# fpusan/moira

Measured on AMD Instinct MI355X. Metric: reads/sec filtered (300 bp synthetic), higher is better.
Workload: dtype f64; 1 GPU; BASELINE configs[1]: 10000000 synthetic single-end 300 bp reads, poisson_binomial filter, alpha 0.005, uncert 0.01, resident in HBM (uint8 10000000 x 320, seed 2); reads_per_gpu=10000000, read_length=300, row_stride=320, parallelism=host-side split, 1 rank(s), no data-path collective, world_size=1, mode=bit-exact (no FMA)

## Files before the change

### include/moira_pb.h

```cpp
#ifndef MOIRA_PB_H
#define MOIRA_PB_H

#include <stdint.h>

#ifdef __cplusplus
extern "C" {
#endif
#if defined(__GNUC__) || defined(__clang__)
#pragma GCC visibility push(default)
#endif

#define MPB_OK            0
#define MPB_E_INVALID    -1
#define MPB_E_NODEVICE   -2
#define MPB_E_HIP        -3
#define MPB_E_NOMEM      -4
#define MPB_E_RANGE      -5

#define MPB_AMBIG_TREAT_AS_ERRORS 0
#define MPB_AMBIG_IGNORE          1
#define MPB_AMBIG_DISALLOW        2

#define MPB_FLAG_ROUND      1u
#define MPB_FLAG_FAST_FMA   2u
#define MPB_FLAG_ODDS      128u
#define MPB_FLAG_DECISION_ONLY 8u
#define MPB_FLAG_TEST_UNDERPREDICT 4u
#define MPB_FLAG_COUNT_CELLS 32u
#define MPB_FLAG_BATCHED_ONLY 16u

#define MPB_FLAG_NO_NARROW 64u
#define MPB_FLAG_NARROW_ROWS(r) (((uint32_t)(r) & 15u) << 8)

#define MPB_FLAG_NARROW_SPLIT(c) (((uint32_t)(c) & 255u) << 12)

#define MPB_FLAG_ODDS_NARROW (1u << 20)

#define MPB_FLAG_POISSON_DEVICE_TAIL (1u << 21)

#define MPB_K_PREPASS   0
#define MPB_K_SCAN      1
#define MPB_K_SCATTER   2
#define MPB_K_DP        3
#define MPB_K_OVERFLOW  4
#define MPB_K_LAMBDA    5
#define MPB_K_WIDE      6
#define MPB_K_NARROW    7
#define MPB_K_FALLBACK  8
#define MPB_K_SAMPLE    9
#define MPB_K_POISSON_TAIL 10
#define MPB_K_PACK_TEXT 11
#define MPB_K_CONTIG    12
#define MPB_K_CONTIG_ROWS 13
#define MPB_K_BGZF_DEFLATE 14
#define MPB_K_BGZF_SCAN  15
#define MPB_K_BGZF_FRAME 16
#define MPB_K_BGZF_INFLATE 17
#define MPB_K_FQ_LINES  18
#define MPB_K_FQ_SCAN   19
#define MPB_K_FQ_STARTS 20
#define MPB_K_FQ_ROWS   21
#define MPB_K_COUNT     22

typedef struct mpb_ctx mpb_ctx;

typedef struct mpb_filter_params {
    double   alpha;
    double   uncert;
    double   maxerrors;
    int32_t  ambig_mode;
    uint32_t flags;
} mpb_filter_params;

typedef struct mpb_filter_counts {
    int64_t n_reads;
    int64_t n_pass;
    int64_t n_fail;
    int64_t n_overflow;
} mpb_filter_counts;

const char *mpb_version(void);
const char *mpb_last_error(void);
int mpb_device_count(void);

int mpb_create(int device_id, mpb_ctx **out);
int mpb_destroy(mpb_ctx *ctx);
int mpb_host_lut(double *a_out, double *b_out);
int mpb_device_lut(mpb_ctx *ctx, double *a_out, double *b_out);
int mpb_stream(mpb_ctx *ctx, void **stream_out);
int mpb_synchronize(mpb_ctx *ctx);

int mpb_malloc(mpb_ctx *ctx, int64_t bytes, void **dptr_out);
int mpb_free(mpb_ctx *ctx, void *dptr);
int mpb_memcpy_h2d(mpb_ctx *ctx, void *dst_dev, const void *src_host, int64_t bytes);
int mpb_memcpy_d2h(mpb_ctx *ctx, void *dst_host, const void *src_dev, int64_t bytes);
int mpb_memset(mpb_ctx *ctx, void *dst_dev, int value, int64_t bytes);
int mpb_host_alloc(mpb_ctx *ctx, int64_t bytes, void **hptr_out);
int mpb_host_free(mpb_ctx *ctx, void *hptr);

int mpb_pack_read(const char *seq, const int32_t *quals, int32_t len,
                  uint8_t *row_out, int32_t row_bytes);
int mpb_pack_read_ascii(const char *seq, const char *qual_ascii, int32_t len,
                        int32_t offset, uint8_t *row_out, int32_t row_bytes);

int mpb_pack_batch_ascii(const char *seq_cat, const char *qual_cat, const int64_t *off, int64_t n,
                         int32_t fastq_offset, int32_t max_len, int64_t row_stride,
                         uint8_t *out, int32_t *lens_out);

int mpb_decode_ascii_device(mpb_ctx *ctx, const uint8_t *d_seq, const uint8_t *d_qual_ascii, int64_t n,
                            int64_t row_stride, const int32_t *d_len, int32_t fixed_len,
                            int32_t fastq_offset, uint8_t *d_q_out, int32_t *d_err);

int mpb_encode_ascii_device(mpb_ctx *ctx, const uint8_t *d_q, int64_t n, int64_t row_stride, int32_t fastq_offset,
                            uint8_t *d_seq_out, uint8_t *d_qual_out);

#define MPB_IDX_SEQ_OFF  2
#define MPB_IDX_QUAL_OFF 4
#define MPB_IDX_QUAL_LEN 5
#define MPB_IDX_COLS     6

typedef struct mpb_text_row { int64_t seq_off, qual_off; int32_t len, pad; } mpb_text_row;
// ... 206 lines not shown
```

### moira_amd/_lib.py

```python
import ctypes as C
import os

_HERE = os.path.dirname(os.path.abspath(__file__))
LIB_PATH = os.path.join(_HERE, "libmoira_pb.so")

MAX_LEN = 65535
OK, E_INVALID, E_NODEVICE, E_HIP, E_NOMEM, E_RANGE = 0, -1, -2, -3, -4, -5
AMBIG = {"treat_as_errors": 0, "ignore": 1, "disallow": 2}
FLAG_ROUND, FLAG_FAST_FMA, FLAG_TEST_UNDERPREDICT, FLAG_DECISION_ONLY, FLAG_BATCHED_ONLY, FLAG_COUNT_CELLS = 1, 2, 4, 8, 16, 32
FLAG_NO_NARROW = 64
FLAG_ODDS = 128
FLAG_ODDS_NARROW = 1 << 20
FLAG_POISSON_DEVICE_TAIL = 1 << 21


def FLAG_NARROW_ROWS(r):
    return (int(r) & 15) << 8


K_PREPASS, K_SCAN, K_SCATTER, K_DP, K_OVERFLOW, K_LAMBDA, K_WIDE, K_NARROW, K_FALLBACK, K_SAMPLE = 0, 1, 2, 3, 4, 5, 6, 7, 8, 9
K_POISSON_TAIL = 10
K_PACK_TEXT = 11
KERNEL_NAMES = {K_PREPASS: "prepass", K_SCAN: "scan", K_SCATTER: "scatter", K_DP: "dp", K_OVERFLOW: "overflow", K_LAMBDA: "lambda",
                K_WIDE: "wide", K_NARROW: "narrow", K_FALLBACK: "fallback", K_SAMPLE: "sample", K_POISSON_TAIL: "poisson_tail",
                K_PACK_TEXT: "pack_text"}
K_CONTIG, K_CONTIG_ROWS = 12, 13
CONTIG_KERNEL_NAMES = {K_CONTIG: "contig", K_CONTIG_ROWS: "contig_rows"}
K_BGZF_DEFLATE, K_BGZF_SCAN, K_BGZF_FRAME = 14, 15, 16
BGZF_KERNEL_NAMES = {K_BGZF_DEFLATE: "bgzf_deflate", K_BGZF_SCAN: "bgzf_scan", K_BGZF_FRAME: "bgzf_frame"}
K_BGZF_INFLATE = 17
INFLATE_KERNEL_NAMES = {K_BGZF_INFLATE: "bgzf_inflate"}
K_FQ_LINES, K_FQ_SCAN, K_FQ_STARTS, K_FQ_ROWS = 18, 19, 20, 21
INDEX_KERNEL_NAMES = {K_FQ_LINES: "fq_lines", K_FQ_SCAN: "fq_scan", K_FQ_STARTS: "fq_starts", K_FQ_ROWS: "fq_rows"}
FQ_WHY = ("taken", "non-ASCII byte", "lone carriage return", "line table", "row check")
BGZF_WHY = ("ok", "header", "block type", "stored length", "code-length code", "repeat", "tree", "symbol", "distance", "overrun",
            "short", "truncated", "trailing bytes", "crc")
BGZF_DATA = 0xff00


class MoiraPBError(RuntimeError):
    pass


class NoDeviceError(MoiraPBError):
    pass


class FilterParams(C.Structure):
    _fields_ = [("alpha", C.c_double), ("uncert", C.c_double), ("maxerrors", C.c_double),
                ("ambig_mode", C.c_int32), ("flags", C.c_uint32)]


class PathInfo(C.Structure):
    _fields_ = [("narrow_rows", C.c_int32), ("sampled", C.c_int32), ("n_fallback", C.c_int64),
                ("sample_hist", C.c_int32 * 16), ("narrow_split", C.c_int32), ("narrow_waves", C.c_int32)]


class FilterCounts(C.Structure):
    _fields_ = [("n_reads", C.c_int64), ("n_pass", C.c_int64), ("n_fail", C.c_int64),
                ("n_overflow", C.c_int64)]


class TextRow(C.Structure):
    _fields_ = [("seq_off", C.c_int64), ("qual_off", C.c_int64), ("len", C.c_int32), ("pad", C.c_int32)]


class PairRow(C.Structure):
    _fields_ = [("fseq_off", C.c_int64), ("fqual_off", C.c_int64), ("fhdr_off", C.c_int64), ("rseq_off", C.c_int64),
                ("rqual_off", C.c_int64), ("l1", C.c_int32), ("l2", C.c_int32), ("hdr_len", C.c_int32), ("pad", C.c_int32)]


class ContigParams(C.Structure):
    _fields_ = [(k, C.c_int32) for k in ("match", "mismatch", "gap", "insert", "deltaq", "consensus", "qscore_cap", "trim_overlap")]


class BgzfStats(C.Structure):
    _fields_ = [(k, C.c_int64) for k in ("members", "dynamic", "fixed", "stored", "literals", "matches", "matched_bytes")]


class BgzfMemberRow(C.Structure):
    _fields_ = [("stream_off", C.c_int64), ("out_off", C.c_int64), ("stream_len", C.c_int32), ("out_len", C.c_int32)]


class BgzfInflateStats(C.Structure):
    _fields_ = [(k, C.c_int64) for k in ("members", "taken", "handed_back", "stored_blocks", "fixed_blocks", "dynamic_blocks",
                                         "literals", "matches", "matched_bytes", "longest_code")]


CONTIG_MAX_LEN = 384

_VP, _I32P, _U8P, _DP = C.c_void_p, C.POINTER(C.c_int32), C.POINTER(C.c_uint8), C.POINTER(C.c_double)
PROTOTYPES = {
    "mpb_version": (C.c_char_p, []),
    "mpb_last_error": (C.c_char_p, []),
    "mpb_device_count": (C.c_int, []),
    "mpb_create": (C.c_int, [C.c_int, C.POINTER(_VP)]),
# ... 136 lines not shown
```

### moira_amd/build.py

```python
import fcntl
import hashlib
import os
import subprocess
import sys

HERE = os.path.dirname(os.path.abspath(__file__))
ROOT = os.path.dirname(HERE)
CSRC = os.path.join(HERE, "csrc")
LIB = os.path.join(HERE, "libmoira_pb.so")
HOST_SOURCES = [os.path.join(CSRC, name) for name in ("mpb_hostonly.cpp", "mpb_context.cpp", "mpb_resident.cpp", "mpb_hostfed.cpp",
                                                      "mpb_perread.cpp", "mpb_poisson.cpp", "mpb_text.cpp", "mpb_contig.cpp",
                                                      "mpb_bgzf.cpp", "mpb_inflate.cpp", "mpb_index.cpp", "mpb_broker.cpp")]
CONTIG_KERNELS = os.path.join(CSRC, "mpb_contig_kernels.hip")
BGZF_KERNELS = os.path.join(CSRC, "mpb_bgzf_kernels.hip")
INFLATE_KERNELS = os.path.join(CSRC, "mpb_inflate_kernels.hip")
INDEX_KERNELS = os.path.join(CSRC, "mpb_index_kernels.hip")
SOURCES = [os.path.join(CSRC, "mpb_kernels.hip"), CONTIG_KERNELS, BGZF_KERNELS, INFLATE_KERNELS, INDEX_KERNELS] + HOST_SOURCES
DEPS = SOURCES + [os.path.join(CSRC, "mpb_internal.h"), os.path.join(CSRC, "mpb_host_internal.h"),
                  os.path.join(CSRC, "mpb_shared.h"), os.path.join(CSRC, "mpb_hostonly.h"), os.path.join(CSRC, "mpb_ctx.h"),
                  os.path.join(CSRC, "mpb_dp_tiles.inc"),
                  os.path.join(CSRC, "mpb_narrow_ring.inc"), os.path.join(CSRC, "mpb_narrow_rs.inc"),
                  os.path.join(CSRC, "mpb_narrow_rg.inc"),
                  os.path.join(CSRC, "mpb_contig_lane.inc"), os.path.join(CSRC, "mpb_contig_args.h"),
                  os.path.join(CSRC, "mpb_contig_rows.inc"),
                  os.path.join(CSRC, "mpb_bgzf_lane.inc"),
                  os.path.join(CSRC, "mpb_inflate_lane.inc"),
                  os.path.join(CSRC, "mpb_index_lane.inc"),
                  os.path.join(CSRC, "contig_posterior.h"),
                  os.path.join(CSRC, "libmoira_pb.map"),
                  os.path.join(ROOT, "include", "moira_pb.h"),
                  os.path.join(ROOT, "include", "mpb_synth.h")]
HIPCC = os.environ.get("HIPCC", "/opt/rocm/bin/hipcc")
FLAGS = ["-O3", "--offload-arch=gfx950", "-fPIC", "-shared", "-std=c++17",
         "-ffp-contract=off", "-fno-fast-math", "-pthread", "-Wall", "-Wno-unused-function",
         "-Werror=pass-failed",
         "-fvisibility=hidden",
         "-Wl,--version-script=" + os.path.join(CSRC, "libmoira_pb.map"),
         "-x", "hip"]


CONTIG_LIB = os.path.join(HERE, "libmoira_contig.so")
CONTIG_SRC = os.path.join(CSRC, "contig.cpp")
CXX = os.environ.get("CXX", "g++")


CONTIG_DEPS = [CONTIG_SRC, os.path.join(CSRC, "contig_posterior.h"), os.path.join(ROOT, "include", "moira_contig.h"),
               os.path.join(ROOT, "include", "moira_io.h")]


def _digest(paths, flags):
    h = hashlib.sha256(" ".join(flags).encode())
    for p in paths:
        with open(p, "rb") as f:
            h.update(f.read())
    return h.hexdigest()


def _is_stale(lib, deps, flags):
    stamp = lib + ".stamp"
    if not os.path.exists(lib) or not os.path.exists(stamp):
        return True
    try:
        return open(stamp).read().strip() != _digest(deps, flags)
    except OSError:
        return True


def _locked_build(lib, deps, flags, cmd, force, verbose):
    with open(lib + ".lock", "w") as lk:
        fcntl.flock(lk, fcntl.LOCK_EX)
        try:
            if force or _is_stale(lib, deps, flags):
                if verbose:
                    print(" ".join(cmd))
                tmp = lib + ".tmp.%d" % os.getpid()
                subprocess.check_call(cmd[:-1] + [tmp])
                os.replace(tmp, lib)
                with open(lib + ".stamp", "w") as f:
                    f.write(_digest(deps, flags))
                if verbose:
                    print("%s: COMPILED now (sources + flags digest %s)" % (os.path.basename(lib), _digest(deps, flags)[:16]))
            elif verbose:
                print("%s: up to date" % os.path.basename(lib))
        finally:
            fcntl.flock(lk, fcntl.LOCK_UN)
    return lib


def report(lib, deps, flags):
    state = "STALE" if _is_stale(lib, deps, flags) else "up to date: its stamp equals the digest of its sources + flags"
    print("%s: %s (digest %s, %d bytes)" % (os.path.basename(lib), state, _digest(deps, flags)[:16],
                                            os.path.getsize(lib) if os.path.exists(lib) else 0))


CONTIG_FLAGS = ["-O3", "-fPIC", "-shared", "-std=c++17", "-ffp-contract=off", "-pthread", "-Wall"]


def contig_stale():
    return _is_stale(CONTIG_LIB, CONTIG_DEPS, CONTIG_FLAGS)


def build_contig(force=False, verbose=False):
    if not force and not contig_stale():
        return CONTIG_LIB
    cmd = [CXX] + CONTIG_FLAGS + [CONTIG_SRC, "-o", CONTIG_LIB]
# ... 46 lines not shown
```

### moira_amd/csrc/mpb_kernels.hip

```cpp

#include "mpb_internal.h"
#include <cstdlib>
#include <cstdio>
#include "../../include/mpb_synth.h"

#pragma clang fp contract(off)

__shared__ double2 mpb_s_lut[256];
__shared__ unsigned long long mpb_s_cells;

namespace {

__constant__ MpbClass c_classes[MPB_NCLS] = MPB_CLASS_TABLE;

struct ClassOfRows {
    uint8_t t[MPB_TILE_MAX_ROWS + 1];
    constexpr ClassOfRows() : t{}
    {
        constexpr MpbClass cl[MPB_NCLS] = MPB_CLASS_TABLE;
        for (int rows = 0; rows < MPB_TILE_MAX_ROWS + 1; rows++) {
            int c = 0;
            for (int k = 0; k < MPB_NCLS - 1; k++) c += (rows > cl[k].cap) ? 1 : 0;
            t[rows] = (uint8_t)c;
        }
// ... 1656 lines not shown
        js = hit ? r : js;
        acc = na;
    }
    if (!(js >= 0 && p0 >= 0x1p-900)) return false;
    e = mpb_add_ns(prm, cross_ee_odds(true, js, prm.thr, p0, lo, hi), nsv);
    if (mode_unsure(prm, e, li)) return false;
    keep = mpb_round_and_keep(prm, e, nsv > 0, li);
    return true;
}

template <int AR = MPB_AR_EXACT, int R>
__device__ __forceinline__ NarRead nar_finish(double (&v)[R], uint32_t &nonzero, const MpbDevParams &prm, bool valid, bool good,
                                              int li, int64_t i, int32_t *my_seg, int &nlist, int lane)
{
    NarRead o;
    if constexpr (AR == MPB_AR_ODDS) {
        o.nsv = li - (int)nonzero;
        o.done = good && nar_odds_result(v, prm, o.nsv, li, o.e, o.keep);
    } else {
    double acc = 0.0, lo = 0.0, hi = 0.0;
    int js = -1;
#pragma unroll
    for (int r = 0; r < R; r++) {
        const double na = acc + v[r];
        const bool hit = (js < 0) && (na > prm.thr);
        lo = hit ? acc : lo;
        hi = hit ? na : hi;
        js = hit ? r : js;
        acc = na;
    }
    o.done = good && js >= 0;
    o.nsv = li - (int)nonzero;
    if (o.done) o.keep = read_result(prm, true, js, lo, hi, o.nsv, o.nsv > 0, li, o.e);
    }
    const unsigned long long todo = __ballot(valid && !o.done);
    if (todo) {
        if (valid && !o.done) my_seg[nlist + __popcll(todo & ((1ull << lane) - 1ull))] = (int32_t)i;
        nlist += __popcll(todo);
    }
#pragma unroll
    for (int r = 0; r < R; r++) v[r] = r == 0 ? 1.0 : 0.0;
    nonzero = 0;
    return o;
}

#define MPB_NRS_TILE 8192
__device__ __forceinline__ void nar_tile_lane(int lane, int &wr_even, int &wr_odd, int &x0)
{
    const int r8 = lane >> 3, c8 = lane & 7;
    wr_even = r8 * 128 + ((c8 ^ (r8 >> 1)) << 4);
    wr_odd = r8 * 128 + ((c8 ^ (4 + (r8 >> 1))) << 4);
    x0 = lane * 128 + (((lane >> 1) & 7) << 4);
}
__device__ __forceinline__ void nar_tile_write(uint8_t *tile, int wr_even, int wr_odd, const u32x4 (&pre)[8])
{
#pragma unroll
    for (int j = 0; j < 8; j++) *reinterpret_cast<u32x4 *>(tile + j * 1024 + ((j & 1) ? wr_odd : wr_even)) = pre[j];
}
__device__ __forceinline__ void nar_tile_fence()
{
    __builtin_amdgcn_fence(__ATOMIC_RELEASE, "wavefront");
    __builtin_amdgcn_wave_barrier();
    __builtin_amdgcn_fence(__ATOMIC_ACQUIRE, "wavefront");
}


#define MPB_NAR_AR MPB_AR_EXACT
#define MPB_NAR_RLO RLO

template <int R, int D>
__global__ __launch_bounds__(256) void k_narrow(const uint8_t *__restrict__ q, int64_t n, int64_t stride, int32_t li,
                                                MpbDevParams prm, const double2 *__restrict__ lut_g,
                                                double *__restrict__ ee, int32_t *__restrict__ ns, uint8_t *__restrict__ pass,
                                                int32_t *__restrict__ seg, int32_t *__restrict__ wave_count)
#include "mpb_narrow_ring.inc"

template <int R, bool ALIGNED>
__global__ __launch_bounds__(256) void k_narrow_rs(const uint8_t *__restrict__ q, int64_t n, int64_t stride, int32_t li, int32_t k,
                                                   MpbDevParams prm, const double2 *__restrict__ lut_g,
                                                   double *__restrict__ ee, int32_t *__restrict__ ns, uint8_t *__restrict__ pass,
                                                   int32_t *__restrict__ seg, int32_t *__restrict__ wave_count)
#include "mpb_narrow_rs.inc"

#define MPB_RG_WIN 4096
#define MPB_RG_BINS 64

__device__ __forceinline__ int rg_group_cost(int chunks) { return chunks + ((chunks + 7) >> 3) + 2; }

__device__ __forceinline__ uint32_t rg_block_excl_scan(uint32_t x, uint32_t *s_wave, int tid)
{
    const int lane = tid & 63, w = tid >> 6;
    uint32_t incl = x;
#pragma unroll
    for (int off = 1; off < 64; off <<= 1) {
        const uint32_t y = __shfl_up(incl, off);
        if (lane >= off) incl += y;
    }
    if (lane == 63) s_wave[w] = incl;
    __syncthreads();
    uint32_t base = 0;
#pragma unroll
    for (int k = 0; k < 3; k++) base += k < w ? s_wave[k] : 0;
    __syncthreads();
    return base + incl - x;
}

__global__ __launch_bounds__(256) void k_rag_sort(const int32_t *__restrict__ len, int64_t n, int32_t max_len, int key_shift,
                                                  int32_t split, int32_t low_pct,
                                                  int2 *__restrict__ ord, int32_t *__restrict__ gpre,
                                                  unsigned long long *__restrict__ wsum)
{
    __shared__ __attribute__((aligned(16))) uint16_t s_cnt[8 * 256];
    __shared__ __attribute__((aligned(16))) uint16_t s_idx[2][MPB_RG_WIN];
    __shared__ __attribute__((aligned(16))) uint16_t s_len[MPB_RG_WIN];
    __shared__ uint32_t s_wave[4];
    const int tid = threadIdx.x, lane = tid & 63, w = tid >> 6;
    const int64_t w0 = (int64_t)blockIdx.x * MPB_RG_WIN;
    const int m = (int)min((int64_t)MPB_RG_WIN, n - w0);
#pragma unroll
    for (int k = 0; k < 16; k++) {
        const int i = k * 256 + tid;
        const int l = i < m ? len[w0 + i] : 0;
        s_len[i] = (uint16_t)((l < 0 || l > max_len) ? 0xffff : l);
    }
    __syncthreads();
    auto key_of = [key_shift](uint32_t l) { return l == 0xffffu ? 0u : ((l + 15u) >> 4) >> key_shift; };
    uint32_t el[16];
    {
        const u32x4 a = *reinterpret_cast<const u32x4 *>(s_len + 16 * tid), b = *reinterpret_cast<const u32x4 *>(s_len + 16 * tid + 8);
        const uint32_t ww[8] = {a.x, a.y, a.z, a.w, b.x, b.y, b.z, b.w};
#pragma unroll
        for (int e = 0; e < 8; e++) { el[2 * e] = key_of(ww[e] & 0xffffu); el[2 * e + 1] = key_of(ww[e] >> 16); }
    }
    const int mine = min(16, max(0, m - 16 * tid));
#pragma unroll
    for (int pass = 0; pass < 2; pass++) {
        if (pass == 1) {
            __syncthreads();
            const u32x4 a = *reinterpret_cast<const u32x4 *>(s_idx[0] + 16 * tid), b = *reinterpret_cast<const u32x4 *>(s_idx[0] + 16 * tid + 8);
            const uint32_t ww[8] = {a.x, a.y, a.z, a.w, b.x, b.y, b.z, b.w};
#pragma unroll
            for (int e = 0; e < 8; e++) { el[2 * e] = ww[e] & 0xffffu; el[2 * e + 1] = ww[e] >> 16; }
        }
        unsigned long long c_lo = 0, c_hi = 0;
#pragma unroll
        for (int r = 0; r < 16; r++) {
            const int d = pass == 0 ? (int)(el[r] & 7u) : (int)(el[r] >> 12);
            const unsigned long long inc = r < mine ? 1ull << (16 * (d & 3)) : 0ull;
            c_lo += (d & 4) ? 0ull : inc;
            c_hi += (d & 4) ? inc : 0ull;
        }
#pragma unroll
        for (int d = 0; d < 8; d++) s_cnt[d * 256 + tid] = (uint16_t)(((d & 4) ? c_hi : c_lo) >> (16 * (d & 3)));
        __syncthreads();
        u32x4 c4 = *reinterpret_cast<const u32x4 *>(s_cnt + 8 * tid);
        uint32_t cc[8] = {c4.x & 0xffffu, c4.x >> 16, c4.y & 0xffffu, c4.y >> 16, c4.z & 0xffffu, c4.z >> 16, c4.w & 0xffffu, c4.w >> 16};
        uint32_t sum = 0;
#pragma unroll
        for (int e = 0; e < 8; e++) sum += cc[e];
        uint32_t run = rg_block_excl_scan(sum, s_wave, tid);
#pragma unroll
        for (int e = 0; e < 8; e++) { const uint32_t c = cc[e]; cc[e] = run; run += c; }
        c4.x = cc[0] | (cc[1] << 16); c4.y = cc[2] | (cc[3] << 16); c4.z = cc[4] | (cc[5] << 16); c4.w = cc[6] | (cc[7] << 16);
        *reinterpret_cast<u32x4 *>(s_cnt + 8 * tid) = c4;
        __syncthreads();
        unsigned long long p_lo = 0, p_hi = 0;
// ... 154 lines not shown
        s_tab[tid] = make_float2(p, tid == 0 ? MPB_MARK_UPPER : tid == 255 ? MPB_MARK_LOWER : p * (1.0f - p));
        const float r = p / (1.0f - p);
        s_pow[tid] = make_float4(log1pf(-p), r, r * r, r * r * r);
    }
    __syncthreads();
    const int k = blockIdx.x * 4 + w;
    if (k >= n_sample) return;
    const int64_t step = n / n_sample;
    const int64_t i = min(n - 1, (int64_t)k * step + (int64_t)(mpb_mix64((uint64_t)k) % (uint64_t)step));
    const int li_raw = len ? len[i] : fixed_len;
    const bool bad_len = li_raw < 0 || li_raw > prm.max_len;
    const int li = bad_len ? 0 : li_raw;
    float mu = 0.f, var = 0.f, k3 = 0.f;
    float lp0 = 0.f, t1 = 0.f, t2 = 0.f, t3 = 0.f;
    int ambi = 0, lower = 0;
    for (int c0 = 0; c0 * 16 < li; c0 += 64 * 15) {
        f32x2 a01 = {0.f, 0.f};
        float s3 = 0.f;
        for (int c = c0 + lane; c * 16 < li && c < c0 + 64 * 15; c += 64) {
            uint4 y = *reinterpret_cast<const uint4 *>(q + i * stride + (int64_t)c * 16);
            const int nv = li - c * 16;
            y.x = fill_dword(y.x, nv); y.y = fill_dword(y.y, nv - 4);
            y.z = fill_dword(y.z, nv - 8); y.w = fill_dword(y.w, nv - 12);
            pre_chunk(s_tab, y, a01, s3);
            const uint32_t ww[4] = {y.x, y.y, y.z, y.w};
#pragma unroll
            for (int d = 0; d < 4; d++)
#pragma unroll
                for (int t = 0; t < 4; t++) {
                    const float4 e = s_pow[(ww[d] >> (8 * t)) & 0xffu];
                    lp0 += e.x; t1 += e.y; t2 += e.z; t3 += e.w;
                }
        }
        const float n255 = floorf(a01.y * (1.0f / MPB_MARK_LOWER));
        const float rem = a01.y - MPB_MARK_LOWER * n255;
        const float nzero = floorf(rem * (1.0f / MPB_MARK_UPPER));
        const float pvar = rem - MPB_MARK_UPPER * nzero;
        mu += a01.x; var += pvar; k3 += pvar - 2.0f * s3;
        ambi += (int)nzero + (int)n255;
        lower += (int)n255;
    }
#pragma unroll
    for (int off = 1; off <= 32; off <<= 1) {
        mu += __shfl_xor(mu, off); var += __shfl_xor(var, off);
        k3 += __shfl_xor(k3, off); ambi += __shfl_xor(ambi, off); lower += __shfl_xor(lower, off);
        lp0 += __shfl_xor(lp0, off); t1 += __shfl_xor(t1, off);
        t2 += __shfl_xor(t2, off); t3 += __shfl_xor(t3, off);
    }
    if (lane == 0) {
        const float vv = fmaxf(var, 1e-12f);
        const float x = mu + prm.z * sqrtf(vv) + (k3 / vv) * prm.zq;
        int rows = (int)floorf(fminf(x, 1e9f) + 0.5f) + 1;
        rows = max(rows, 5);
        const float thr = (float)prm.thr;
        const float p0 = __expf(lp0);
        const float e1 = t1, e2 = 0.5f * (t1 * t1 - t2), e3 = (t1 * t1 * t1 - 3.0f * t1 * t2 + 2.0f * t3) * (1.0f / 6.0f);
        float cdf = p0;
        if (cdf > thr) rows = 1;
        else if ((cdf += p0 * e1) > thr) rows = 2;
        else if ((cdf += p0 * e2) > thr) rows = 3;
        else if ((cdf += p0 * e3) > thr) rows = 4;
        rows = max(min(rows, li - ambi + 1), 1);
        atomicAdd(hist + ((lower > 0 || bad_len) ? 0 : min(rows, MPB_NAR_BUCKETS - 1)),
                  len ? max(1, (li + 15) >> 4) : 1);
        if (len && lower == 0 && !bad_len) {
            if (rows >= 3) atomicMin(hist + MPB_NAR_BUCKETS, (li + 15) >> 4);
            if (rows >= 4) atomicMin(hist + MPB_NAR_BUCKETS + 1, (li + 15) >> 4);
        }
    }
}

}

static inline int pre_blocks(int64_t n) { return (int)((n + MPB_PRE_READS - 1) / MPB_PRE_READS); }

void mpb_launch_prepass(const uint8_t *q, int64_t n, int64_t stride, const int32_t *len,
                        const MpbDevParams &prm, const MpbWorkspace &ws, int32_t *ns_out,
                        double *ee_out, uint8_t *pass_out, hipStream_t s, const int32_t *list)
{
#define MPB_PRE_LAUNCH(RG, LG, LS)                                                                                      \
    hipLaunchKernelGGL((k_prepass<RG, LG, LS>), dim3(pre_blocks(n)), dim3(256), 0, s, q, n, stride, len, prm, o, ws.blockhist, list)
    const PreOut o = {ws.cls, ns_out, ee_out, pass_out, ws.bad_len, ws.wide_list, ws.wide_rows, ws.wide_count};
    const bool long_rows = prm.max_len > 16 * 12 * MPB_PRE_NB;
    if (list) {
        if (len) { if (long_rows) MPB_PRE_LAUNCH(true, true, true); else MPB_PRE_LAUNCH(true, false, true); }
        else     { if (long_rows) MPB_PRE_LAUNCH(false, true, true); else MPB_PRE_LAUNCH(false, false, true); }
    } else {
        if (len) { if (long_rows) MPB_PRE_LAUNCH(true, true, false); else MPB_PRE_LAUNCH(true, false, false); }
        else     { if (long_rows) MPB_PRE_LAUNCH(false, true, false); else MPB_PRE_LAUNCH(false, false, false); }
    }
#undef MPB_PRE_LAUNCH
}

void mpb_launch_decode_classify(const uint8_t *seq, const uint8_t *qual, int32_t offset, uint8_t *out, int32_t *err,
                                int64_t n, int64_t stride, const int32_t *len, const MpbDevParams &prm,
                                const MpbWorkspace &ws, int32_t *ns_out, double *ee_out, uint8_t *pass_out, hipStream_t s)
{
    const PreOut o = {ws.cls, ns_out, ee_out, pass_out, ws.bad_len, ws.wide_list, ws.wide_rows, ws.wide_count};
    const PreDecode dec = {seq, qual, out, offset, err};
    const uint8_t *q = out;
    const uint32_t cpr = (uint32_t)(stride >> 4);
    const uint32_t magic = cpr == 1 ? 0u : (uint32_t)(((1ull << 32) + cpr - 1) / cpr);
    if (len) hipLaunchKernelGGL((k_classify_linear<true, true>), dim3(pre_blocks(n)), dim3(256), 0, s, q, n, stride, len, prm, o, ws.blockhist, dec, magic);
    else     hipLaunchKernelGGL((k_classify_linear<false, true>), dim3(pre_blocks(n)), dim3(256), 0, s, q, n, stride, len, prm, o, ws.blockhist, dec, magic);
}

void mpb_launch_encode(const uint8_t *q, int64_t n, int64_t stride, int32_t offset, uint8_t *seq, uint8_t *qual, hipStream_t s)
{
    const int64_t chunks = n * (stride / 16);
    hipLaunchKernelGGL(k_encode_ascii, dim3((unsigned)((chunks + 255) / 256)), dim3(256), 0, s, q, n, stride, offset, seq, qual);
}

void mpb_launch_scan(int64_t n, const int32_t *len, const MpbWorkspace &ws, hipStream_t s)
{
    const int nb = len ? MPB_LEN_BINS : 1;
    hipLaunchKernelGGL(k_scan, dim3(MPB_NCLS * nb), dim3(256), 0, s, ws.blockhist, pre_blocks(n), ws.tables);
    hipLaunchKernelGGL(k_tables, dim3(1), dim3(512), 0, s, ws.tables, nb, ws.ovf_count, ws.pass_count);
}

void mpb_launch_scatter(int64_t n, const int32_t *len, const int32_t *ns, const MpbDevParams &prm, const MpbWorkspace &ws,
                        hipStream_t s, const int32_t *list)
{
    if (len)
        hipLaunchKernelGGL((k_scatter<true>), dim3(pre_blocks(n)), dim3(256), 0, s, ws.cls, n, len, prm.max_len, prm.len_shift,
                           ws.blockhist, ws.tables, ns, ws.perm, ws.perm_ns, list);
    else
        hipLaunchKernelGGL((k_scatter<false>), dim3(pre_blocks(n)), dim3(256), 0, s, ws.cls, n, len, prm.max_len, prm.len_shift,
                           ws.blockhist, ws.tables, ns, ws.perm, ws.perm_ns, list);
}

#define MPB_DP_GRID (1 << 20)


static DpArgs make_args(const uint8_t *q, int64_t stride, const int32_t *len, const MpbDevParams &prm,
                        const MpbWorkspace &ws, const int32_t *ns, double *ee, uint8_t *pass, int final_pass)
{
    DpArgs A;
    A.q = q; A.stride = stride; A.len = len; A.ns = ns; A.cls = ws.cls; A.ee = ee; A.pass = pass;
    A.ovf_list = ws.ovf_list; A.ovf_count = ws.ovf_count; A.alg_cells = ws.alg_cells; A.prm = prm; A.final_pass = final_pass;
    A.perm = ws.perm; A.perm_ns = final_pass == 0 ? ws.perm_ns : nullptr;
    return A;
}

void mpb_launch_dp(const uint8_t *q, int64_t n, int64_t stride, const int32_t *len,
                   const MpbDevParams &prm, const MpbWorkspace &ws, const int32_t *ns,
                   double *ee, uint8_t *pass, hipStream_t s, const double2 *lut_odds)
{
    const int64_t tiles = (n + 63) / 64 + MPB_NCLS;
    const int chunk_tiles = tiles >= 32768 ? MPB_DP_CHUNK : tiles >= 16384 ? 4 : tiles >= 8192 ? 2 : 1;
    constexpr int grid_cap = MPB_DP_GRID;
    int64_t want = (tiles + 4 * chunk_tiles - 1) / (4 * chunk_tiles);
    const int blocks = (int)(want < grid_cap ? (want > 0 ? want : 1) : grid_cap);
    DpArgs A = make_args(q, stride, len, prm, ws, ns, ee, pass, 0);
    if (lut_odds)
        hipLaunchKernelGGL(k_dp_odds, dim3(blocks), dim3(256), 0, s, A, lut_odds, ws.tables, ws.perm, chunk_tiles);
    else if (prm.flags & MPB_FLAG_FAST_FMA)
        hipLaunchKernelGGL((k_dp<true, false>), dim3(blocks), dim3(256), 0, s, A, ws.lut, ws.tables, ws.perm, chunk_tiles);
    else
        hipLaunchKernelGGL((k_dp<false, false>), dim3(blocks), dim3(256), 0, s, A, ws.lut, ws.tables, ws.perm, chunk_tiles);
}

#define MPB_WIDE_GRID 1024

template <bool FINAL>
static void launch_wide(const DpArgs &A, const double2 *lut, const int32_t *list, const int32_t *budget,
                        const int32_t *count, int max_rows, hipStream_t s)
// ... 258 lines not shown
```

### moira_amd/engine.py

```python
import ctypes as C
import math

import numpy as np

from . import _lib as L


def _round_up(x, m):
    return (x + m - 1) // m * m


class DeviceBuffer:

    def __init__(self, engine, nbytes):
        self.engine, self.nbytes = engine, int(nbytes)
        p = C.c_void_p()
        L.check(engine.lib.mpb_malloc(engine.ctx, self.nbytes, C.byref(p)))
        self.ptr = p.value

    def upload(self, arr):
        arr = np.ascontiguousarray(arr)
        assert arr.nbytes <= self.nbytes
        L.check(self.engine.lib.mpb_memcpy_h2d(self.engine.ctx, self.ptr, arr.ctypes.data, arr.nbytes))
        return self
# ... 102 lines not shown
    return rows


class ContigResult:
    __slots__ = ("cbuf", "cidx", "aux", "done", "rec_cap", "n_done", "n_handed_back", "aln", "aln_len", "score")

    def __init__(self, *a):
        for k, v in zip(self.__slots__, a):
            setattr(self, k, v)


class ContigFilterResult(ContigResult):
    __slots__ = ("ee", "ns", "passed", "lens", "has_n", "filtered", "n_pass", "n_overflow", "filter_error")

    def __init__(self, contigs, *a):
        for k in ContigResult.__slots__:
            setattr(self, k, getattr(contigs, k))
        for k, v in zip(ContigFilterResult.__slots__, a):
            setattr(self, k, v)


def check_host_batch(q, lens, fixed_len, out, limit):
    q = np.ascontiguousarray(q, dtype=np.uint8)
    if q.ndim != 2:
        raise ValueError("q must be a 2-D (reads x stride) uint8 matrix")
    n, stride = q.shape
    if lens is not None:
        lens = np.ascontiguousarray(lens, dtype=np.int32)
        if lens.shape != (n,):
            raise ValueError("lens must have one entry per read")
        if n and (lens.min() < 0 or lens.max() > stride):
            raise ValueError("a length does not fit the row stride")
        if n and limit is not None and lens.max() > limit:
            raise ValueError("reads longer than %d bases are not supported (longest: %d)" % (limit, int(lens.max())))
    elif fixed_len is None:
        raise ValueError("give lens or fixed_len")
    if out is None:
        res = np.empty(n, np.float64), np.empty(n, np.int32), np.empty(n, np.uint8)
    else:
        ee, ns, ps = out
        if (ee.dtype, ns.dtype, ps.dtype) != (np.float64, np.int32, np.uint8) or \
                not (len(ee) >= n and len(ns) >= n and len(ps) >= n) or \
                not (ee.flags.c_contiguous and ns.flags.c_contiguous and ps.flags.c_contiguous):
            raise ValueError("out must be contiguous (float64, int32, uint8) arrays of at least n entries")
        res = ee[:n], ns[:n], ps[:n]
    return q, n, stride, lens, res


class Engine:

    batched_only = False

    def __init__(self, device=0):
        self.lib = L.load()
        ctx = C.c_void_p()
        L.check(self.lib.mpb_create(int(device), C.byref(ctx)))
        self.ctx = ctx
        self.device = int(device)
        self._pinned = {}

    def close(self):
        if getattr(self, "ctx", None):
            for p in list(getattr(self, "_pinned", {}).values()):
                self.lib.mpb_host_free(self.ctx, p)
            self._pinned = {}
            self.lib.mpb_destroy(self.ctx)
            self.ctx = None

    def __del__(self):
        try:
            self.close()
        except Exception:
            pass

    def __enter__(self):
        return self

    def __exit__(self, *a):
        self.close()

    @staticmethod
    def params(alpha=0.005, uncert=0.01, maxerrors=None, ambigs="treat_as_errors", round_=False,
               fast_fma=False, test_underpredict=False, decision_only=False, batched_only=False, count_cells=False,
               no_narrow=False, narrow_rows=0, narrow_split=0, odds=False, odds_narrow=False, poisson_device_tail=False):
        if ambigs not in L.AMBIG:
            raise ValueError("ambigs must be one of %s" % sorted(L.AMBIG))
        if odds and fast_fma:
            raise ValueError("odds and fast_fma are two arithmetics for the same pass: set one")
        if odds_narrow and not odds:
            raise ValueError("odds_narrow needs odds=True (MPB_FLAG_ODDS_NARROW needs MPB_FLAG_ODDS)")
        flags = (L.FLAG_ROUND if round_ else 0) | (L.FLAG_FAST_FMA if fast_fma else 0) | \
                (L.FLAG_TEST_UNDERPREDICT if test_underpredict else 0) | \
                (L.FLAG_DECISION_ONLY if decision_only else 0) | \
                (L.FLAG_BATCHED_ONLY if batched_only else 0) | (L.FLAG_COUNT_CELLS if count_cells else 0) | \
                (L.FLAG_NO_NARROW if no_narrow else 0) | (L.FLAG_ODDS if odds else 0) | \
                (L.FLAG_ODDS_NARROW if odds_narrow else 0) | (L.FLAG_POISSON_DEVICE_TAIL if poisson_device_tail else 0) | \
                L.FLAG_NARROW_ROWS(narrow_rows) | ((int(narrow_split) & 255) << 12)
        return L.FilterParams(float(alpha), float(uncert),
                              math.nan if maxerrors is None else float(maxerrors),
                              L.AMBIG[ambigs], flags)

    def alloc(self, nbytes):
        return DeviceBuffer(self, nbytes)

    def host_alloc(self, shape, dtype=np.uint8):
        shape = (int(shape),) if np.isscalar(shape) else tuple(int(x) for x in shape)
        dt = np.dtype(dtype)
        nbytes = int(np.prod(shape)) * dt.itemsize
        p = C.c_void_p()
        L.check(self.lib.mpb_host_alloc(self.ctx, nbytes, C.byref(p)))
        buf = (C.c_uint8 * max(nbytes, 1)).from_address(p.value)
        arr = np.frombuffer(buf, dtype=dt, count=int(np.prod(shape))).reshape(shape)
        self._pinned[arr.ctypes.data] = p.value
        return arr

    def host_free(self, arr):
        p = self._pinned.pop(arr.ctypes.data, None)
        if p is not None and self.ctx:
            L.check(self.lib.mpb_host_free(self.ctx, p))

    def synchronize(self):
        L.check(self.lib.mpb_synchronize(self.ctx))

    def stream(self):
        p = C.c_void_p()
        L.check(self.lib.mpb_stream(self.ctx, C.byref(p)))
        return p.value

    def pack(self, seqs, quals, stride=None):
        n = len(quals)
        lens = np.array([len(x) for x in quals], np.int32)
        if stride is None:
            stride = _round_up(max(int(lens.max()) if n else 1, 1), 16)
        q = np.zeros((n, stride), np.uint8)
        for i in range(n):
            qi = np.ascontiguousarray(quals[i], dtype=np.int32)
            s = seqs[i] if seqs is not None else None
            if s is not None:
                if len(s) != len(qi):
                    raise ValueError("contig and contig_quals must have the same length")
                s = s.encode() if isinstance(s, str) else s
            L.check(self.lib.mpb_pack_read(s, qi.ctypes.data, len(qi), q[i].ctypes.data, stride))
        return q, lens

    def pack_batch_ascii(self, seqs, qual_strs, fastq_offset=33, stride=None, max_len=0):
        n = len(qual_strs)
        off = np.zeros(n + 1, np.int64)
        if n:
            off[1:] = np.cumsum([len(x) for x in qual_strs])
        lens_full = off[1:] - off[:-1]
        longest = int(min(lens_full.max(), max_len) if (n and max_len > 0) else (lens_full.max() if n else 1))
        if stride is None:
            stride = _round_up(max(longest, 1), 16)
        q = np.empty((n, stride), np.uint8)
        lens = np.empty(n, np.int32)
        if seqs is not None and any(len(s) != len(x) for s, x in zip(seqs, qual_strs)):
            raise ValueError("contig and contig_quals must have the same length")
        L.check(self.lib.mpb_pack_batch_ascii("".join(seqs).encode() if seqs is not None else None,
                                              "".join(qual_strs).encode("latin-1"), off.ctypes.data, n,
                                              int(fastq_offset), int(max_len), stride, q.ctypes.data,
                                              lens.ctypes.data))
        return q, lens

    @staticmethod
    def text_rows(idx, sel=None, text_bytes=0, max_len=0, stride=0):
        return text_rows(idx, sel, text_bytes, max_len, stride)

    def pack_text_device(self, d_text, text_bytes, d_rows, n, stride, d_q_out, d_len_out, d_flags_out=None, d_status=None,
                         fastq_offset=33, lower_n_is_base=False):
        ptr = lambda b: (b.ptr if isinstance(b, DeviceBuffer) else b)
        L.check(self.lib.mpb_pack_text_device(self.ctx, ptr(d_text), int(text_bytes), ptr(d_rows), int(n), int(fastq_offset),
                                              1 if lower_n_is_base else 0, int(stride), ptr(d_q_out), ptr(d_len_out),
                                              ptr(d_flags_out) if d_flags_out is not None else None, ptr(d_status)))

    def filter_text(self, buf, idx, sel=None, fastq_offset=33, max_len=0, lower_n_is_base=False, poisson=False, out=None, **kw):
        params = kw.pop("params", None) or self.params(**kw)
        idx, sel, n = _index_args(idx, sel)
        keep, addr, nbytes = _text_ptr(buf)
        if out is None:
# ... 366 lines not shown
```

Baseline: 2.572 billion reads/s.

## Add cache-line panel prepass kernel for fixed-length strided reads

Adds a new prepass kernel for fixed-length reads whose stride is a multiple of 64 and at most 960 bytes. Each wave loads 128-byte panels of 64 or 128 rows with buffer loads, prefetching the next panel, and transposes them through a swizzled LDS tile so every lane walks one read. This replaces the per-row load pattern of the existing prepass with coalesced full-line loads. Reads containing 255-quality marks are recomputed serially from global memory, and a new flag restores the old row-based prepass.

```diff
diff --git a/include/moira_pb.h b/include/moira_pb.h
--- a/include/moira_pb.h
+++ b/include/moira_pb.h
@@ -37,6 +37,8 @@
 #define MPB_FLAG_ODDS_NARROW (1u << 20)
 
 #define MPB_FLAG_POISSON_DEVICE_TAIL (1u << 21)
+
+#define MPB_FLAG_PREPASS_ROWS (1u << 22)
 
 #define MPB_K_PREPASS   0
 #define MPB_K_SCAN      1
diff --git a/moira_amd/_lib.py b/moira_amd/_lib.py
--- a/moira_amd/_lib.py
+++ b/moira_amd/_lib.py
@@ -12,6 +12,8 @@
 FLAG_ODDS = 128
 FLAG_ODDS_NARROW = 1 << 20
 FLAG_POISSON_DEVICE_TAIL = 1 << 21
+
+FLAG_PREPASS_ROWS = 1 << 22
 
 
 def FLAG_NARROW_ROWS(r):
diff --git a/moira_amd/build.py b/moira_amd/build.py
--- a/moira_amd/build.py
+++ b/moira_amd/build.py
@@ -20,7 +20,7 @@
                   os.path.join(CSRC, "mpb_shared.h"), os.path.join(CSRC, "mpb_hostonly.h"), os.path.join(CSRC, "mpb_ctx.h"),
                   os.path.join(CSRC, "mpb_dp_tiles.inc"),
                   os.path.join(CSRC, "mpb_narrow_ring.inc"), os.path.join(CSRC, "mpb_narrow_rs.inc"),
-                  os.path.join(CSRC, "mpb_narrow_rg.inc"),
+                  os.path.join(CSRC, "mpb_narrow_rg.inc"), os.path.join(CSRC, "mpb_prepass_lines.inc"),
                   os.path.join(CSRC, "mpb_contig_lane.inc"), os.path.join(CSRC, "mpb_contig_args.h"),
                   os.path.join(CSRC, "mpb_contig_rows.inc"),
                   os.path.join(CSRC, "mpb_bgzf_lane.inc"),
diff --git a/moira_amd/csrc/mpb_kernels.hip b/moira_amd/csrc/mpb_kernels.hip
--- a/moira_amd/csrc/mpb_kernels.hip
+++ b/moira_amd/csrc/mpb_kernels.hip
@@ -1762,6 +1762,11 @@
                                                    int32_t *__restrict__ seg, int32_t *__restrict__ wave_count)
 #include "mpb_narrow_rs.inc"
 
+template <int K>
+__global__ __launch_bounds__(256) void k_prepass_lines(const uint8_t *__restrict__ q, int64_t n, int64_t stride,
+                                                       MpbDevParams prm, PreOut o, int32_t *__restrict__ blockhist)
+#include "mpb_prepass_lines.inc"
+
 #define MPB_RG_WIN 4096
 #define MPB_RG_BINS 64
 
@@ -2082,6 +2087,11 @@
     hipLaunchKernelGGL((k_prepass<RG, LG, LS>), dim3(pre_blocks(n)), dim3(256), 0, s, q, n, stride, len, prm, o, ws.blockhist, list)
     const PreOut o = {ws.cls, ns_out, ee_out, pass_out, ws.bad_len, ws.wide_list, ws.wide_rows, ws.wide_count};
     const bool long_rows = prm.max_len > 16 * 12 * MPB_PRE_NB;
+    if (!len && !list && stride % 64 == 0 && stride <= 960 && !(prm.flags & MPB_FLAG_PREPASS_ROWS)) {
+        if (stride % 128 == 0) hipLaunchKernelGGL((k_prepass_lines<1>), dim3(pre_blocks(n)), dim3(256), 0, s, q, n, stride, prm, o, ws.blockhist);
+        else                   hipLaunchKernelGGL((k_prepass_lines<2>), dim3(pre_blocks(n)), dim3(256), 0, s, q, n, stride, prm, o, ws.blockhist);
+        return;
+    }
     if (list) {
         if (len) { if (long_rows) MPB_PRE_LAUNCH(true, true, true); else MPB_PRE_LAUNCH(true, false, true); }
         else     { if (long_rows) MPB_PRE_LAUNCH(false, true, true); else MPB_PRE_LAUNCH(false, false, true); }
diff --git a/moira_amd/csrc/mpb_prepass_lines.inc b/moira_amd/csrc/mpb_prepass_lines.inc
--- /dev/null
+++ b/moira_amd/csrc/mpb_prepass_lines.inc
@@ -0,0 +1,151 @@
+{
+    __shared__ float2 s_tab[256];
+    __shared__ __attribute__((aligned(128))) uint8_t s_tile[4][MPB_NRS_TILE];
+    __shared__ int s_hist[MPB_NCLS];
+    const int tid = threadIdx.x, lane = tid & 63;
+    const int w = __builtin_amdgcn_readfirstlane(tid >> 6);
+    {
+        const bool amb = tid == 0 || tid == 255;
+        float p = __builtin_amdgcn_exp2f(-0.33219281f * (float)tid);
+        p = amb ? 0.0f : p;
+        s_tab[tid] = make_float2(p, tid == 0 ? MPB_MARK_UPPER : tid == 255 ? MPB_MARK_LOWER : p * (1.0f - p));
+    }
+    if (tid < MPB_NCLS) s_hist[tid] = 0;
+    __syncthreads();
+
+    constexpr int rows_sb = 64 * K;
+    const int istride = __builtin_amdgcn_readfirstlane((int)stride);
+    const int KB = K * istride;
+    const int NP = KB >> 7;
+    const int li = prm.fixed_len, lend = max(li, 1);
+    const int64_t wave_row0 = (int64_t)blockIdx.x * MPB_PRE_READS + w * 256;
+    const int nsb = wave_row0 >= n ? 0 : (int)min((int64_t)(256 / rows_sb), (n - wave_row0 + rows_sb - 1) / rows_sb);
+    const int total = nsb * NP;
+    uint8_t *const tile = s_tile[w];
+    const int r8 = lane >> 3, c8 = lane & 7;
+    const int voff = r8 * KB + c8 * 16;
+    int wr_even, wr_odd, x0;
+    nar_tile_lane(lane, wr_even, wr_odd, x0);
+
+    u32x4 pre[8];
+    auto load_panel = [&](const int sb, const int pk) {
+        const int64_t first = wave_row0 + (int64_t)sb * rows_sb;
+        const uint64_t base = (uint64_t)(uintptr_t)q + (uint64_t)first * (uint64_t)stride;
+        const int64_t rows_here = (n - first) < rows_sb ? (n - first) : rows_sb;
+        const uint32_t b_lo = (uint32_t)__builtin_amdgcn_readfirstlane((int)(uint32_t)base);
+        const uint32_t b_hi = (uint32_t)__builtin_amdgcn_readfirstlane((int)(uint32_t)(base >> 32));
+        const uint32_t b_n = (uint32_t)__builtin_amdgcn_readfirstlane((int)(uint32_t)(rows_here * stride));
+        const __amdgpu_buffer_rsrc_t rsrc = __builtin_amdgcn_make_buffer_rsrc(
+            (void *)(uintptr_t)(((uint64_t)b_hi << 32) | b_lo), 0, (int)b_n, 0x00020000);
+#pragma unroll
+        for (int j = 0; j < 8; j++) pre[j] = __builtin_amdgcn_raw_buffer_load_b128(rsrc, voff, j * 8 * KB + pk * 128, 0);
+    };
+    int pf_sb = 0, pf_pk = 0, cur_sb = 0, cur_pk = 0;
+    if (total > 0) {
+        load_panel(pf_sb, pf_pk);
+        if (++pf_pk == NP) { pf_pk = 0; pf_sb++; }
+    }
+
+    float mu = 0.f, var = 0.f, k3 = 0.f, s3 = 0.f;
+    f32x2 a01 = {0.f, 0.f};
+    uint32_t ambi = 0;
+    int u = 0, sread = 0;
+
+    auto peel = [&]() {
+        const float n255 = floorf(a01.y * (1.0f / MPB_MARK_LOWER));
+        const float rem = a01.y - MPB_MARK_LOWER * n255;
+        const float nzero = floorf(rem * (1.0f / MPB_MARK_UPPER));
+        const float pvar = rem - MPB_MARK_UPPER * nzero;
+        mu += a01.x;
+        var += pvar;
+        k3 += pvar - 2.0f * s3;
+        ambi += (uint32_t)nzero + ((uint32_t)n255 << 16);
+        a01 = (f32x2){0.f, 0.f};
+        s3 = 0.f;
+    };
+    float r_mu[4], r_var[4], r_k3[4];
+    uint32_t r_ambi[4];
+#pragma unroll
+    for (int s = 0; s < 4; s++) { r_mu[s] = r_var[s] = r_k3[s] = 0.f; r_ambi[s] = 0; }
+    auto finish = [&](const int slot) {
+#pragma unroll
+        for (int s = 0; s < 4; s++)
+            if (slot == s) { r_mu[s] = mu; r_var[s] = var; r_k3[s] = k3; r_ambi[s] = ambi; }
+        mu = var = k3 = 0.f;
+        ambi = 0;
+    };
+
+    for (int t = 0; t < total; t++) {
+        nar_tile_write(tile, wr_even, wr_odd, pre);
+        nar_tile_fence();
+        if (t + 1 < total) {
+            load_panel(pf_sb, pf_pk);
+            if (++pf_pk == NP) { pf_pk = 0; pf_sb++; }
+        }
+        __builtin_amdgcn_sched_barrier(0);
+#pragma unroll
+        for (int h = 0; h < 2; h++) {
+            const int nb = li - u;
+            if (nb >= 64) {
+#pragma unroll
+                for (int c = 0; c < 4; c++) {
+                    const u32x4 x = *reinterpret_cast<const u32x4 *>(tile + (x0 ^ ((h * 4 + c) << 4)));
+                    pre_chunk(s_tab, make_uint4(x.x, x.y, x.z, x.w), a01, s3);
+                }
+            } else if (nb > 0) {
+#pragma unroll
+                for (int c = 0; c < 4; c++) {
+                    const int nv = nb - 16 * c;
+                    if (nv <= 0) break;
+                    const u32x4 x = *reinterpret_cast<const u32x4 *>(tile + (x0 ^ ((h * 4 + c) << 4)));
+                    uint4 y = make_uint4(x.x, x.y, x.z, x.w);
+                    if (nv < 16) {
+                        y.x = fill_dword(y.x, nv); y.y = fill_dword(y.y, nv - 4);
+                        y.z = fill_dword(y.z, nv - 8); y.w = fill_dword(y.w, nv - 12);
+                    }
+                    pre_chunk(s_tab, y, a01, s3);
+                }
+            }
+            const bool ends = u < lend && lend <= u + 64;
+            if (h == 1 || ends) peel();
+            if (ends) finish(cur_sb * K + sread);
+            u += 64;
+            if (u == istride) { u = 0; sread++; }
+        }
+        if (++cur_pk == NP) { cur_pk = 0; cur_sb++; sread = 0; }
+        nar_tile_fence();
+    }
+#pragma unroll 1
+    for (int slot = 0; slot < nsb * K; slot++) {
+        const int sr = slot % K;
+        const int64_t i = wave_row0 + (int64_t)(slot / K) * rows_sb + (int64_t)lane * K + sr;
+        if (i >= n) continue;
+#pragma unroll
+        for (int s = 0; s < 4; s++)
+            if (slot == s) { mu = r_mu[s]; var = r_var[s]; k3 = r_k3[s]; ambi = r_ambi[s]; }
+        if (ambi >> 16) {
+            const uint8_t *src = q + i * stride;
+            mu = var = k3 = 0.f;
+            a01 = (f32x2){0.f, 0.f};
+            s3 = 0.f;
+#pragma unroll 1
+            for (int c0 = 0; c0 < li; c0 += 16) {
+#pragma unroll 1
+                for (int d = 0; d < 4; d++)
+                    pre_dword_again(s_tab, fill_dword(*reinterpret_cast<const uint32_t *>(src + c0 + d * 4), li - c0 - 4 * d), a01, s3);
+                if (((sr * istride + c0 + 16) & 127) == 0 || c0 + 16 >= li) {
+                    const float nzero = floorf(a01.y * (1.0f / MPB_MARK_UPPER));
+                    const float pvar = a01.y - MPB_MARK_UPPER * nzero;
+                    mu += a01.x;
+                    var += pvar;
+                    k3 += pvar - 2.0f * s3;
+                    a01 = (f32x2){0.f, 0.f};
+                    s3 = 0.f;
+                }
+            }
+        }
+        class_read(i, mu, var, k3, ambi, li, false, false, prm, o, s_hist, 1);
+    }
+    __syncthreads();
+    if (tid < MPB_NCLS) blockhist[(int64_t)tid * gridDim.x + blockIdx.x] = s_hist[tid];
+}
diff --git a/moira_amd/engine.py b/moira_amd/engine.py
--- a/moira_amd/engine.py
+++ b/moira_amd/engine.py
@@ -208,7 +208,8 @@
     @staticmethod
     def params(alpha=0.005, uncert=0.01, maxerrors=None, ambigs="treat_as_errors", round_=False,
                fast_fma=False, test_underpredict=False, decision_only=False, batched_only=False, count_cells=False,
-               no_narrow=False, narrow_rows=0, narrow_split=0, odds=False, odds_narrow=False, poisson_device_tail=False):
+               no_narrow=False, narrow_rows=0, narrow_split=0, odds=False, odds_narrow=False, poisson_device_tail=False,
+               prepass_rows=False):
         if ambigs not in L.AMBIG:
             raise ValueError("ambigs must be one of %s" % sorted(L.AMBIG))
         if odds and fast_fma:
@@ -221,6 +222,7 @@
                 (L.FLAG_BATCHED_ONLY if batched_only else 0) | (L.FLAG_COUNT_CELLS if count_cells else 0) | \
                 (L.FLAG_NO_NARROW if no_narrow else 0) | (L.FLAG_ODDS if odds else 0) | \
                 (L.FLAG_ODDS_NARROW if odds_narrow else 0) | (L.FLAG_POISSON_DEVICE_TAIL if poisson_device_tail else 0) | \
+                (L.FLAG_PREPASS_ROWS if prepass_rows else 0) | \
                 L.FLAG_NARROW_ROWS(narrow_rows) | ((int(narrow_split) & 255) << 12)
         return L.FilterParams(float(alpha), float(uncert),
                               math.nan if maxerrors is None else float(maxerrors),
```

New measurement: 2.595 billion reads/s, median of 6. Within noise of the previous version (+0.9%).
